# tum-vision/lsd_slam

Measured on AMD Instinct MI355X. Metric: tracked frames/sec (full track+map loop) at 640x480, frames resident in HBM (8-bit upload excluded: value_pcie_inclusive has it), higher is better.
Workload: dtype f32

## Files before the change

lsd_slam_amd/csrc/lsdhip_internal.hpp:

```cpp
#pragma once
#include <hip/hip_runtime.h>
#include <atomic>
#include <chrono>
#include <cmath>
#include <cstddef>
#include <cstdint>
#include <cstdio>
#include <cstring>
#include <mutex>
#include <string>
#include <vector>
#include "../../include/lsdhip.h"

#define LSD_LEVELS LSDHIP_PYRAMID_LEVELS
#define LSD_TRACK_MIN_LEVEL 1
#define LSD_TRACK_MAX_LEVEL 5
#define LSD_QUICK_KF_CHECK_LVL 4

void lsd_set_error(const char* fmt, ...);
#define HIPCHK(expr)                                                                       \
  do {                                                                                     \
    hipError_t e_ = (expr);                                                                \
    if (e_ != hipSuccess) {                                                                \
      lsd_set_error("%s failed: %s (%s:%d)", #expr, hipGetErrorString(e_), __FILE__, __LINE__); \
// ... 49 lines not shown
  TrackLevel lv[LSD_LEVELS];
  uint8_t* wasGood;
  float cameraPixelNoise2, var_weight, huber_half;
  float lambdaSuccessFac, lambdaFailFac;
  int useAffine;
  int lastLevel;
  int topLevel;
  lsdm::SE3fH T0;
  float aff_a0, aff_b0;
  int evalOnly;
  int trackFrameSemantics;
};
struct TrackSpec {
  int specC;
  int specGrid;
  int trials[LSD_LEVELS];
  uint8_t* wasGoodSide;
  unsigned maskStride;
  int seq;
  int copyMask;
  unsigned long long dbgCum;
  unsigned long long* dbgCounters;
  int last;
#ifdef LSD_PHASE_TRACE
  int traceWg;
#endif
#ifdef LSD_DEVTOOLS
  int* dbgLog;
#endif
};

struct TrackState {
  lsdm::SE3fH T;
  lsdm::SE3fH Tn;
  float R[9], t[3];
  float aff_a, aff_b, aff_a_lastIt, aff_b_lastIt;
  float lastErr, LM_lambda, last_residual;
  int level, iteration, incTry, phase;
  int pending;
  float A[36], b[6];
  float inc[6];
  float bytes;
  int done, diverged;
  int numEvaluations, numWarpUpdates;
  float pointUsage, goodCount, badCount, meanRes;
  int levelEvals[LSD_LEVELS];
// ... 414 lines not shown
```

lsd_slam_amd/csrc/track_device.hpp:

```cpp
#pragma once
#include "lsdhip_internal.hpp"
#include <type_traits>

template <int CTRL, int ROW_MASK, int BANK_MASK>
__device__ __forceinline__ float dpp_f(float v) {
  return __builtin_bit_cast(float, __builtin_amdgcn_update_dpp(0, __builtin_bit_cast(int, v), CTRL, ROW_MASK, BANK_MASK, true));
}
__device__ __forceinline__ int dpp_max_i(int a, int b) { return a > b ? a : b; }
template <int CTRL, int ROW_MASK, int BANK_MASK>
__device__ __forceinline__ int dpp_i(int v) {
  return __builtin_amdgcn_update_dpp(-1, v, CTRL, ROW_MASK, BANK_MASK, false);
}
template <int CTRL, int ROW_MASK, int BANK_MASK>
__device__ __forceinline__ int dpp_i0(int v) {
  return __builtin_amdgcn_update_dpp(0, v, CTRL, ROW_MASK, BANK_MASK, true);
}
__device__ __forceinline__ int wave_max_to_lane63(int v) {
  int t = dpp_max_i(v, dpp_i<0x111, 0xf, 0xf>(v));
  t = dpp_max_i(t, dpp_i<0x112, 0xf, 0xf>(v));
  t = dpp_max_i(t, dpp_i<0x113, 0xf, 0xf>(v));
  t = dpp_max_i(t, dpp_i<0x114, 0xf, 0xe>(t));
  t = dpp_max_i(t, dpp_i<0x118, 0xf, 0xc>(t));
  t = dpp_max_i(t, dpp_i<0x142, 0xa, 0xf>(t));
  t = dpp_max_i(t, dpp_i<0x143, 0xc, 0xf>(t));
// ... 400 lines not shown
  float tot[RS_NUM];
};
struct LmPar {
  float lambdaInitial, stepSizeMin, convergenceEps, minWarped, lambdaSuccessFac, lambdaFailFac;
  int maxIts, w, h, writeMask, evalOnly, useAffine, tfSemantics, lastLevel, trials;
};
__device__ __forceinline__ void stage_lm_par(const TrackJob& job, int level, LmPar& p, const int trials = 1) {
  const TrackLevel& L = job.lv[level];
  LmPar v;
  v.lambdaInitial = L.lambdaInitial; v.stepSizeMin = L.stepSizeMin; v.convergenceEps = L.convergenceEps; v.minWarped = L.minWarped;
  v.lambdaSuccessFac = job.lambdaSuccessFac; v.lambdaFailFac = job.lambdaFailFac;
  v.maxIts = L.maxIts; v.w = L.w; v.h = L.h; v.writeMask = L.writeMask; v.evalOnly = job.evalOnly; v.useAffine = job.useAffine;
  v.tfSemantics = job.trackFrameSemantics; v.lastLevel = job.lastLevel;
  v.trials = trials;
  p = v;
}

#ifdef LSD_PHASE_TRACE
#define LM_MARK(k) do { if (trp && lane == 0) trp[k] = clock64(); } while (0)
#else
#define LM_MARK(k) do { } while (0)
#endif
__device__ __forceinline__ float lm_werr(float sumWeightedErr, int M) { return sumWeightedErr * frcp((float)((M >> 2) << 2)); }
__device__ __forceinline__ float lm_lambda_fail(float LM_lambda, int incTry, float lambdaFailFac) {
  if (LM_lambda == 0) return 0.2f;
  double p = 1.0;
  for (int i = 0; i < incTry; i++) p *= (double)lambdaFailFac;
  return (float)((double)LM_lambda * p);
}
__device__ __forceinline__ float eval_bytes(const float N, const LmPar& L) {
  const float wh = (float)L.w * (float)L.h;
  const float texels = 4.0f * N < wh ? 4.0f * N : wh;
  return 20.0f * N + (L.writeMask ? 5.0f * N : 0.0f) + 12.0f * texels;
}
__device__ __forceinline__ float inc_norm2(const float* inc) {
  const float i0 = inc[0], i1 = inc[1], i2 = inc[2], i3 = inc[3], i4 = inc[4], i5 = inc[5];
  return (i0 * i0 + (i1 * i1 + i2 * i2)) + (i3 * i3 + (i4 * i4 + i5 * i5));
}
template <bool SPEC = false>
__device__ __forceinline__ bool lm_wave(const LmPar& par, TrackState& S, const float col, LmShared& sh, const int lane,
                                        TrackSummary* out, unsigned long long* trp, const int consumed = 0, const int mycand = 0, const int doneWord = 1) {
  float* const tot = sh.tot;
  S.lastCand = consumed;
  S.ncand = 1;
  const LmPar L = par;
  const int maxIts = L.maxIts;
  const int M = (int)rl(col, RS_M);
  const float refNum = rl(col, RS_NREF);
  const float goodCount = rl(col, RS_GOOD), badCount = rl(col, RS_BAD);
  float aff_a_lastIt, aff_b_lastIt;
  {
// ... 8 lines not shown
  S.meanRes = rl(col, RS_SUMSIGNED) * frcp(goodCount);
  S.aff_a_lastIt = aff_a_lastIt;
  S.aff_b_lastIt = aff_b_lastIt;
  S.numEvaluations = S.numEvaluations + 1;
  if (lane == 0) S.levelEvals[S.level] = S.levelEvals[S.level] + 1;
  S.bytes = S.bytes + eval_bytes(refNum, L);
  S.pending = 0;
  LM_MARK(12);
  if (L.evalOnly) { S.done = 1; if (out && lane == 0) write_summary(S, tot, out, doneWord); return false; }

  if (M < L.minWarped) {
    S.diverged = 1; S.done = 1;
    if (out && lane == 0) write_summary(S, tot, out, doneWord);
    return false;
  }
  const float werr = lm_werr(rl(col, RS_WERR), M);
  const bool useAffine = L.useAffine != 0;
  const bool tfSemantics = L.tfSemantics != 0;

  float LM_lambda = S.LM_lambda, lastErr = S.lastErr;
  int iteration = S.iteration, incTry = S.incTry;
  lsdm::SE3fH T = S.T;
  bool propose = false, start_iteration = false, accepted = false, rejected = false;
  if (S.phase == 0) {
    accepted = true;
    lastErr = werr;
    LM_lambda = L.lambdaInitial;
    iteration = 0;
    start_iteration = true;
  } else {
    const float error = werr;
    if (error < lastErr) {
      accepted = true;
      T = S.Tn;
      S.T = T;
      if (error > L.convergenceEps * lastErr) iteration = maxIts;
      lastErr = error;
      if (tfSemantics) S.last_residual = error;
      if (LM_lambda <= 0.2) LM_lambda = 0;
      else LM_lambda *= L.lambdaSuccessFac;
      iteration++;
      start_iteration = true;
    } else {
      if (!(inc_norm2(S.inc) > L.stepSizeMin)) {
        iteration = maxIts;
        iteration++;
        start_iteration = true;
      } else {
        LM_lambda = lm_lambda_fail(LM_lambda, incTry, L.lambdaFailFac);
        propose = true;
        rejected = true;
      }
    }
  }
  if (accepted) {
    if (useAffine) { S.aff_a = aff_a_lastIt; S.aff_b = aff_b_lastIt; }
    const float rn = frcp((float)((size_t)6 * (size_t)(M >> 2)));
    const int k = lane - RS_A0;
    if (k >= 0 && k < 21) {
      const int i = (k >= 6) + (k >= 11) + (k >= 15) + (k >= 18) + (k >= 20);
      const int j = k - (i * 6 - (i * (i - 1)) / 2) + i;
      const float v = (0.0f + col) * rn;
      S.A[i * 6 + j] = v;
      S.A[j * 6 + i] = v;
    }
    if (lane >= RS_B0 && lane < RS_B0 + 6) S.b[lane - RS_B0] = (0.0f - col) * rn;
  }
  if (start_iteration && iteration < maxIts) { S.numWarpUpdates = S.numWarpUpdates + 1; incTry = 0; propose = true; }
  S.lastErr = lastErr;
  S.LM_lambda = LM_lambda;
  S.iteration = iteration;
  LM_MARK(13);
  if (propose) {
    const int extra = SPEC ? mycand : 0;
    for (int j = 0; j < extra; j++) { incTry++; LM_lambda = lm_lambda_fail(LM_lambda, incTry, L.lambdaFailFac); }
    S.ncand = L.trials;
    float inc[6];
    const float damp = 1 + LM_lambda;
    LM_MARK(14);
    gj6_solve_wave(S.A, S.b, damp, sh.gj, lane, inc);
    LM_MARK(15);
    S.incTry = incTry + 1;
#pragma unroll
    for (int i = 0; i < 6; i++) S.inc[i] = inc[i];
    set_eval_pose(S, se3f_mul_wave(se3f_exp_wave(inc, lane), T, lane));
    S.phase = 1;
    LM_MARK(16);
    return true;
  }
  S.incTry = incTry;
  if (!tfSemantics) S.last_residual = lastErr;
  if (S.level == L.lastLevel) {
    S.done = 1;
    if (out && lane == 0) write_summary(S, tot, out, doneWord);
  } else {
    S.level = S.level - 1;
    S.phase = 0;
    set_eval_pose(S, T);
// ... 126 lines not shown
__device__ __forceinline__ int xcd_tile(int b, int nb) { return (nb & 7) == 0 ? (b & 7) * (nb >> 3) + (b >> 3) : b; }


struct TrialRecord {
  float inc[6];
  float pose[7];
  float R[9], t[3];
  float pad_[7];
};
static_assert(sizeof(TrialRecord) == 128 && sizeof(lsdm::SE3fH) == sizeof(float[7]), "a trial record is 32 floats; its pose is a TrackState::Tn");
enum { TRIAL_RECORD_WORDS = offsetof(TrialRecord, pad_) / 4 };
__device__ __forceinline__ float trial_record_word(const TrackState& S, const int i) {
  constexpr int P = offsetof(TrialRecord, pose) / 4, R = offsetof(TrialRecord, R) / 4, T = offsetof(TrialRecord, t) / 4;
  return i < P ? S.inc[i] : (i < R ? ((const float*)&S.Tn)[i - P] : (i < T ? S.R[i - R] : S.t[i - T]));
}
__device__ __forceinline__ void trial_record_adopt(TrackState& S, const TrialRecord& rec, const int lane) {
  if (lane < 6) S.inc[lane] = rec.inc[lane];
  if (lane < 7) ((float*)&S.Tn)[lane] = rec.pose[lane];
  if (lane < 9) S.R[lane] = rec.R[lane];
  if (lane < 3) S.t[lane] = rec.t[lane];
}
__device__ __forceinline__ int trials_at(const TrackSpec& spec, const int level) { return (spec.specC > 1 && spec.trials[level] > 1) ? spec.trials[level] : 1; }

#define RS_COLS 44
struct TrackScratch {
  float* sums;
  int4* topkey;
  float* topval;
  int max_rows;
  int cmax;
  TrialRecord* recs;
#ifdef LSD_PHASE_TRACE
  unsigned long long* trace;
#endif
};
```

lsd_slam_amd/csrc/tracker.hip:

```cpp
#include <atomic>
#include <chrono>
#include "track_device.hpp"
#include "reposition_plan.hpp"

#ifdef LSD_PHASE_TRACE
#define PHASE_MARK(k) do { if (trOn_ && threadIdx.x == 0) tr_[k] = clock64(); } while (0)
#define LSD_TRACE_WORDS 32
#define TRACE_PARAMS , const bool trOn_, unsigned long long* const tr_
#define TRACE_ARGS , trOn_, tr_
#define TRACE_PUT(rec, who, k, v) do { if (trOn_ && threadIdx.x == (who)) (rec)[k] = (unsigned long long)(v); } while (0)
#define TRACE_LM_REC (trOn_ ? tr_ : nullptr)
__device__ __forceinline__ unsigned long long* trace_open(unsigned long long* trace, const bool mine, unsigned long long** s_trp) {
  if (!mine) return trace;
  const unsigned long long n = trace[0];
  trace[0] = n + 1;
  unsigned long long* tr_ = trace + 1 + (n % 4096) * LSD_TRACE_WORDS;
  for (int k = 0; k < LSD_TRACE_WORDS; k++) tr_[k] = 0;
  tr_[8] = wall_clock64();
  tr_[24] = (unsigned long long)gridDim.x; tr_[25] = (unsigned long long)gridDim.y;
  *s_trp = tr_;
  return tr_;
}
#else
#define PHASE_MARK(k) do { } while (0)
// ... 31 lines not shown
  if (tid < 36) S.A[tid] = 0;
  if (tid < 6) { S.b[tid] = 0; S.inc[tid] = 0; }
}

struct StepAddr {
  const float *sums_in, *topval_in;
  float *sums_out, *topval_out;
  const int4* topkey_in; int4* topkey_out;
  const TrialRecord* recs_in;
  TrialRecord* recs_out;
  int max_rows, cmax;
};
template <bool BATCH, int MODE>
__device__ __forceinline__ StepAddr step_addr(const TrackScratch& sc, const int parity) {
  const size_t rows = (size_t)sc.max_rows, cm = (size_t)sc.cmax, job0 = BATCH ? (size_t)blockIdx.y * 2 * cm : 0;
  const size_t in = job0 + (size_t)parity * cm, out = job0 + (size_t)(MODE == TS_EVAL ? parity : 1 - parity) * cm;
  constexpr size_t TAIL = TAIL_ROWS * TAIL_STRIDE;
  return {sc.sums + in * RS_COLS * rows, sc.topval + in * rows * TAIL, sc.sums + out * RS_COLS * rows, sc.topval + out * rows * TAIL,
          sc.topkey + in * rows, sc.topkey + out * rows, sc.recs + in, sc.recs + out, sc.max_rows, sc.cmax};
}

struct StepRole { int cand, bx; bool leader, leaves; };
template <bool BATCH, int MODE>
__device__ __forceinline__ void step_role(StepRole& r, const TrackJob& job, const TrackSpec& spec, const TrackState& S) {
  const int lvlPending = S.level;
  if (MODE == TS_FUSED) {
    const int nbl = job.lv[lvlPending].nblocks;
    const int tr = trials_at(spec, lvlPending);
    r.cand = (int)blockIdx.x / nbl; r.bx = (int)blockIdx.x - r.cand * nbl;
    const bool needTrial = S.pending ? r.cand < tr : r.cand == 0;
    const bool needNext = S.pending && lvlPending > job.lastLevel && (int)blockIdx.x < job.lv[lvlPending - 1].nblocks;
    r.leaves = !r.leader && !needTrial && !needNext;
  }
  if (BATCH && MODE == TS_LM) {
    r.cand = (int)blockIdx.x; r.bx = 0;
    r.leaves = !r.leader && !(S.pending && r.cand < trials_at(spec, lvlPending));
  }
  if (BATCH && MODE == TS_EVAL) {
    const int nbl = job.lv[lvlPending].nblocks;
    r.cand = (int)blockIdx.x / nbl; r.bx = (int)blockIdx.x - r.cand * nbl;
  }
}

constexpr int STRIP_CHMAX = 8;
__device__ __forceinline__ void strip_request(const TrackLevel& L, const int tile_, const int wave, const int lane, int& cntv, unsigned (&ow)[STRIP_CHMAX]) {
  const int px = L.w * L.h;
  const int base_ = tile_ * L.tilePx;
  const int b0_ = base_ >> 8;
  const int mblk_ = (min(base_ + L.tilePx, px) - base_ + 255) >> 8;
  const gbyte* offs = (const gbyte*)L.kf_refBlk;
  const __attribute__((address_space(1))) int* cnts = (const __attribute__((address_space(1))) int*)(offs + ((size_t)((px + 255) >> 8) << 8));
  cntv = lane < mblk_ ? cnts[b0_ + lane] : 0;
#pragma unroll
  for (int c = 0; c < STRIP_CHMAX; c++) {
    const int blk = c * 4 + wave;
    ow[c] = blk < mblk_ ? *(const __attribute__((address_space(1))) unsigned*)(offs + ((size_t)(b0_ + blk) << 8) + (lane << 2)) : 0u;
  }
}

// ... 166 lines not shown
      a4.w += live ? v[c][q].w : 0.f;
    }
    if (sumLane && base + c < ncandPending) *(float4*)&s_sumT[base + c][slot][c4 * 4] = a4;
  }
}
template <int TRIALS_MAX>
__device__ __forceinline__ void column_sums(const StepAddr& A, const int nb, const int ncandPending, const int t, const SumTable s_sumT) {
  constexpr int NSLOT = SUM_NSLOT, QMAX = SUM_QMAX;
  const int slot_ = t / (RS_COLS / 4); const bool sumLane = slot_ < NSLOT;
  const int slot = sumLane ? slot_ : 0, c4 = sumLane ? t - slot_ * (RS_COLS / 4) : 0;
  const int K = (nb + NSLOT - 1) / NSLOT;
  const float4* p = (const float4*)A.sums_in + c4;
  const size_t trialStrideF4 = (size_t)RS_COLS * A.max_rows / 4;
  if (ncandPending == 1) {
    if (K <= 2) colsum<2, 1>(p, trialStrideF4, nb, ncandPending, 0, slot, c4, sumLane, s_sumT);
    else if (K <= 5) colsum<5, 1>(p, trialStrideF4, nb, ncandPending, 0, slot, c4, sumLane, s_sumT);
    else if (K <= 10) colsum<10, 1>(p, trialStrideF4, nb, ncandPending, 0, slot, c4, sumLane, s_sumT);
    else colsum<QMAX, 1>(p, trialStrideF4, nb, ncandPending, 0, slot, c4, sumLane, s_sumT);
  } else if (K <= 2) colsum<2, TRIALS_MAX>(p, trialStrideF4, nb, ncandPending, 0, slot, c4, sumLane, s_sumT);
  else if (K <= 5) colsum<5, TRIALS_MAX>(p, trialStrideF4, nb, ncandPending, 0, slot, c4, sumLane, s_sumT);
  else if (K <= 10) { for (int base = 0; base < ncandPending; base += 3) colsum<10, 3>(p, trialStrideF4, nb, ncandPending, base, slot, c4, sumLane, s_sumT); }
  else { for (int base = 0; base < ncandPending; base++) colsum<QMAX, 1>(p, trialStrideF4, nb, ncandPending, base, slot, c4, sumLane, s_sumT); }
}
template <int TRIALS_MAX>
struct FinishTables {
  enum { WORDS = TRIALS_MAX * (SUM_NSLOT * RS_COLS + TAIL_ROWS * TAIL_STRIDE + 1) };
  SumTable sum; TailTable sub; int* nsub;
  __device__ __forceinline__ explicit FinishTables(float* buf)
      : sum((SumTable)buf), sub((TailTable)(buf + TRIALS_MAX * SUM_NSLOT * RS_COLS)), nsub((int*)(buf + TRIALS_MAX * (SUM_NSLOT * RS_COLS + TAIL_ROWS * TAIL_STRIDE))) {}
};
__device__ __forceinline__ float slot_total(const SumTable s_sumT, const int c, const int col) {
  float s = s_sumT[c][0][col];
#pragma unroll
  for (int k = 1; k < SUM_NSLOT; k++) s += s_sumT[c][k][col];
  return s;
}

__device__ __forceinline__ int pick_trial(TrackState& S, const LmPar& par, const int level, const int ncandPending, const SumTable s_sumT, const TailTable s_subT,
                                          const int* s_nsubT, const TrialRecord* s_rec, const int tid) {
  if (ncandPending <= 1) return 0;
  const int c = tid < ncandPending ? tid : 0;
  const int Mc = (int)slot_total(s_sumT, c, RS_M);
  const float ws = tail_drop(slot_total(s_sumT, c, RS_WERR), Mc, s_nsubT[c], tail_word(RS_WERR), s_subT[c]);
  const float werrc = lm_werr(ws, Mc);
  const float incdot = inc_norm2(c == 0 ? S.inc : s_rec[c].inc);
  const bool stop = Mc < par.minWarped || werrc < S.lastErr || !(incdot > par.stepSizeMin);
  const unsigned long long sm = __ballot(stop && tid < ncandPending);
  const int pc = sm ? (int)__ffsll((long long)sm) - 1 : ncandPending - 1;
  if (pc > 0) {
    float lam = S.LM_lambda;
    const int it0 = S.incTry;
    for (int j = 0; j < pc; j++) lam = lm_lambda_fail(lam, it0 + j, par.lambdaFailFac);
    const float skipped = eval_bytes(slot_total(s_sumT, 0, RS_NREF), par);
    const float bytes0 = S.bytes;
    const int ne0 = S.numEvaluations, le0 = S.levelEvals[level];
    float bytes1 = bytes0;
    for (int j = 0; j < pc; j++) bytes1 = bytes1 + skipped;
    S.LM_lambda = lam;
    S.incTry = it0 + pc;
    S.numEvaluations = ne0 + pc;
    if (tid == 0) S.levelEvals[level] = le0 + pc;
    S.bytes = bytes1;
    trial_record_adopt(S, s_rec[pc], tid);
  }
  return pc;
}
__device__ __forceinline__ float finish_totals(const SumTable s_sumT, const TailTable s_subT, const int* s_nsubT, const int pc, const int tid) {
  const int M = (int)slot_total(s_sumT, pc, RS_M);
  const float s = tid < RS_END ? slot_total(s_sumT, pc, tid) : 0.f;
  return tail_drop(s, M, s_nsubT[pc], tail_word(tid), s_subT[pc]);
}
template <int BLOCK>
__device__ __forceinline__ void copy_side_mask(const TrackJob& job, const TrackState& S, const TrackSpec& spec, const int level, const int bx, const int nb, const int tid) {
  const uint8_t* side = spec.wasGoodSide + (size_t)(S.lastCand - 1) * spec.maskStride;
  EvalCtx a;
  make_ctx_dev(job, S, level, a);
  const int work = a.npts >= 0 ? a.npts : a.w * a.h;
  for (int i = bx * BLOCK + tid; i < work; i += nb * BLOCK) {
    float px, py, pz, I_ref, var;
    int maskIdx;
    if (fetch_point(a, i, px, py, pz, I_ref, var, maskIdx) && maskIdx >= 0) job.wasGood[maskIdx] = side[maskIdx];
  }
}

template <int BLOCK>
__device__ __forceinline__ void eval_strip(const EvalCtx& a, const int tilePx, const int tile, const int work, const int cntv, const unsigned (&ow)[STRIP_CHMAX],
                                           unsigned* const s_list , gbyte* const wasGood, float (&acc)[RS_END], int& key0, int& key1, int& key2,
                                           const int tid TRACE_PARAMS) {
  const int wave = tid >> 6, lane = tid & 63;
  const int base = tile * tilePx;
  const int stripEnd = min(base + tilePx, work);
  const int b0 = base >> 8;
// ... 45 lines not shown
    stageA(tid, A1);
    stageB(A1, B0);
    stageA(tid + BLOCK, A1);
    PHASE_MARK(22);
    auto stageC = [&](const StB& B) {
      if (B.live) {
        const int x_ = (int)(B.xy & 0xffffu), y_ = (int)(B.xy >> 16);
        visit_point(a, B.q, B.t, B.pz, B.I_ref, B.var, wasGood, __mul24(y_, a.w) + x_, __mul24(x_, a.h) + y_, acc, key0, key1, key2);
      }
    };
    for (int r = 0; r < rounds; r += 2) {
      stageB(A1, B1);
      stageA(tid + (r + 2) * BLOCK, A2);
      stageC(B0);
      stageB(A2, B0);
      stageA(tid + (r + 3) * BLOCK, A1);
      stageC(B1);
    }
  }
  __syncthreads();
}
__device__ __forceinline__ void eval_groups_of_four(const EvalCtx& a, int i, const int stride, const int work, gbyte* const wasGood, float (&acc)[RS_END],
                                                    int& key0, int& key1, int& key2) {
  const int sy = stride / a.w, sx = stride - sy * a.w;
  int x = i % a.w, y = i / a.w;
  struct Pt { int i, x, y; bool valid; RefPlanes r; float img, pz; PointWarp q; PointTexels t; };
  while (i < work) {
    Pt P[4];
#pragma unroll
    for (int k = 0; k < 4; k++) {
      Pt& p = P[k];
      p.i = i; p.x = x; p.y = y;
      p.valid = i < work;
      const int li = p.valid ? i : 0;
      fetch_request(a, li, p.r);
      p.img = a.kf_image[li];
      i += stride; x += sx; y += sy;
      if (x >= a.w) { x -= a.w; y++; }
    }
#pragma unroll
    for (int k = 0; k < 4; k++) {
      Pt& p = P[k];
      float px = 0.f, py = 0.f;
      p.pz = 1.f;
      p.valid = p.valid && ref_pixel_inside(a, p.x, p.y) && fetch_finish(a, p.x, p.y, p.r, px, py, p.pz);
      eval_warp(a, px, py, p.pz, p.q);
      eval_fetch(a, p.q, p.valid && p.q.in_image, p.t);
    }
// ... 15 lines not shown
      if (q.in_image) eval_fetch(a, q, true, t);
      visit_point(a, q, t, pz, I_ref, var, maskIdx >= 0 ? wasGood : nullptr, maskIdx, a.npts >= 0 ? i : (i % a.w) * a.h + (i / a.w), acc, key0, key1, key2);
    }
  }
}

constexpr int RED_NPASS = 1;
constexpr int RED_CPP = (RS_END + RED_NPASS - 1) / RED_NPASS;
template <int BLOCK, bool BATCH, int MODE>
__device__ __forceinline__ void reduce_and_store(const EvalCtx& a, const TrackLevel& L, TrackState& S, const int tile, const float (&acc)[RS_END],
                                                 const int key0, const int key1, const int key2, float* const s_red, float (*const s_sum)[64], int (*const s_wtop)[3],
                                                 int* const s_top, float* const sums_out, int4* const topkey_out, float* const topval_out, const int tid) {
  constexpr int NPASS = RED_NPASS, CPP = RED_CPP;
  constexpr int RSLICE = BLOCK / CPP;
  constexpr int RRUN = (BLOCK + RSLICE - 1) / RSLICE;
  const bool stripRows = BATCH && L.tilePx > 0;
  const bool candLane = tid >= BLOCK - 64 && tid < BLOCK - 61;
  TailCandidate c;
  float cPz = 0.f;
  PointWarp cq; PointTexels ct;
  if (stripRows) {
    block_top3(key0, key1, key2, s_wtop, s_top);
    if (candLane) c.request(a, s_top[tid - (BLOCK - 64)]);
  }
#pragma unroll
  for (int hp = 0; hp < NPASS; hp++) {
    if (hp > 0) __syncthreads();
#pragma unroll
    for (int k = 0; k < CPP; k++)
      if (hp * CPP + k < RS_END) s_red[k * (BLOCK + 1) + tid] = acc[hp * CPP + k];
    __syncthreads();
    if (MODE == TS_FUSED && hp == 0 && tid == 0) { S.pending = 1; S.numLaunches = S.numLaunches + 1; }
    if (stripRows && hp == 0 && candLane && c.key >= 0) {
      float px, py;
      ref_point_at(a, c.x, c.y, c.id, px, py, cPz);
      eval_warp(a, px, py, cPz, cq);
      eval_fetch(a, cq, cq.in_image, ct);
    }
    {
      const int slice = tid / CPP, k = tid - slice * CPP;
      if (slice < RSLICE) s_sum[slice][k] = slice_sum<BLOCK + 1, RRUN>(s_red, k, slice);
    }
    __syncthreads();
    if (stripRows && hp == 0 && candLane) {
      float* row = topval_out + (size_t)(tile * TAIL_ROWS + (tid - (BLOCK - 64))) * TAIL_STRIDE;
      if (c.key >= 0) {
        PointOut o;
        eval_finish(a, cq, ct, cPz, c.img, c.var, o);
        tail_row(o, row);
      }
      ((int*)row)[TAIL_KEY] = c.key;
    }
    if (tid < CPP && hp * CPP + tid < RS_END) {
      float s = s_sum[0][tid];
#pragma unroll
      for (int sl = 1; sl < RSLICE; sl++) s += s_sum[sl][tid];
      sums_out[(size_t)tile * RS_COLS + (hp * CPP + tid)] = s;
    }
  }
  if (!stripRows) block_top3(key0, key1, key2, s_wtop, s_top);
  if (tid == 0) topkey_out[tile] = make_int4(s_top[0], s_top[1], s_top[2], -1);
  if (L.singlePass && key0 >= 0) {
    const int r = key0 == s_top[0] ? 0 : (key0 == s_top[1] ? 1 : (key0 == s_top[2] ? 2 : -1));
    if (r >= 0) tail_row_from_sums(acc, topval_out + (size_t)(tile * TAIL_ROWS + r) * TAIL_STRIDE);
  }
}

#ifdef LSD_ORDER_CHECK
__device__ __forceinline__ void order_check_totals(const TrackSpec& spec, const float s, const int pc, const int tid) {
  unsigned hv = tid < RS_END ? __float_as_uint(s) * (2654435761u * (unsigned)(tid + 1)) : 0u;
  hv += (unsigned)pc * 97u;
  for (int off = 32; off > 0; off >>= 1) hv += __shfl_xor(hv, off);
  if (tid == 0) {
    const unsigned long long slot = 8 + 2 * ((spec.dbgCum / 400ull) % 8192ull);
    __hip_atomic_fetch_min(&spec.dbgCounters[slot], (unsigned long long)hv, __ATOMIC_RELAXED, __HIP_MEMORY_SCOPE_AGENT);
    __hip_atomic_fetch_max(&spec.dbgCounters[slot + 1], (unsigned long long)hv, __ATOMIC_RELAXED, __HIP_MEMORY_SCOPE_AGENT);
  }
}
#endif

__device__ __forceinline__ void warm_job_arguments() {
  typedef const unsigned __attribute__((address_space(4))) cuint;
  cuint* ka = (cuint*)__builtin_amdgcn_kernarg_segment_ptr();
  unsigned warm = 0;
#pragma unroll
  for (int i = 0; i < (int)(sizeof(TrackJob) / 4); i += 32) warm ^= ka[i];
  asm volatile("" ::"s"(warm));
}

template <int BLOCK, bool BATCH, int MODE>
__device__ __forceinline__ void track_step_impl(const TrackJob& jobv, const TrackJob* __restrict__ jobs, TrackState* __restrict__ st2,
                                                TrackScratch sc, TrackSummary* __restrict__ out, int parity, int first, const TrackSpec& spec) {
  const TrackJob& job = BATCH ? jobs[blockIdx.y] : jobv;
  if (!BATCH) warm_job_arguments();
  if (BATCH) { st2 += 2 * (size_t)blockIdx.y; out += blockIdx.y; }
  const StepAddr A = step_addr<BATCH, MODE>(sc, parity);
  constexpr int WAVES = BLOCK / 64, SUMW = WAVES - 1;
  constexpr int NSLICE = (SUMW * 64) / RS_END, CPP = RED_CPP, RSLICE_ = BLOCK / CPP;
  __shared__ TrackState S;
  __shared__ LmShared sh;
  __shared__ LmPar s_par;
  __shared__ float s_sum[(NSLICE > RSLICE_ ? NSLICE : RSLICE_)][64];
  __shared__ __attribute__((aligned(16))) float s_red[CPP * (BLOCK + 1) + 8];
  __shared__ int s_wtop[WAVES][3];
  __shared__ int s_top[3];
  const int tid = threadIdx.x, wave = tid >> 6, lane = tid & 63;
  StepRole role = {0, (int)blockIdx.x, blockIdx.x == 0, false};
  const bool leader = role.leader;
  TrackState* next = st2 + (1 - parity);
  constexpr int TRIALS_MAX = BATCH ? (MODE == TS_EVAL ? 1 : LSD_BATCH_SPEC_MAX) : LSD_SPEC_MAX;
  constexpr bool SPEC_LM = MODE != TS_EVAL;
  static_assert(FinishTables<TRIALS_MAX>::WORDS <= CPP * (BLOCK + 1) + 8, "the finishing phase's tables must fit the reduction buffer");
  const FinishTables<TRIALS_MAX> ft(s_red);
  __shared__ TrialRecord s_rec[TRIALS_MAX];
#ifdef LSD_PHASE_TRACE
  __shared__ unsigned long long* s_trp;
  const bool trOn_ = sc.trace != nullptr && (int)blockIdx.x == (BATCH ? spec.traceWg : 0) && (!BATCH || blockIdx.y == 0);
  unsigned long long* const tr_ = trace_open(sc.trace, trOn_ && tid == 0, &s_trp);
#endif
  PHASE_MARK(0);
  if (!BATCH && MODE == TS_FUSED && !first && !leader && st2[parity].done) return;
  if (!BATCH && MODE == TS_FUSED && leader && tid == 0 && spec.seq != 0) out->seq = spec.seq;
  if (first) {
    track_state_begin(S, job, tid);
  } else {
    copy_words<sizeof(TrackState) / 4>(&S, st2 + parity, tid, BLOCK);
    if (SPEC_LM && A.cmax > 1 && tid < (int)(sizeof(s_rec) / 4)) ((float*)s_rec)[tid] = ((const float*)A.recs_in)[tid < (int)(sizeof(TrialRecord) / 4) * A.cmax ? tid : 0];
  }
  __syncthreads();
  PHASE_MARK(1);
#ifdef LSD_DEVTOOLS
  const int lvlIn_ = S.level, numLaunchesIn_ = S.numLaunches, pendingIn_ = S.pending, ncandIn_ = S.ncand;
#endif
  if (S.done) {
    LAUNCH_LOG(1, pendingIn_, ncandIn_, -1);
    if (MODE != TS_EVAL && leader) { copy_words<sizeof(TrackState) / 4>(next, &S, tid, BLOCK); }
    return;
  }
  const int lvlPending = S.level;
  const int doneWord = (MODE == TS_FUSED && spec.seq != 0) ? (BATCH ? spec.seq : (spec.seq >> 12)) : 1;
  step_role<BATCH, MODE>(role, job, spec, S);
  if (role.leaves) return;
  int cand = role.cand, bx = role.bx;

  int cntv = 0;
  unsigned ow[STRIP_CHMAX];
  bool havePre = false;
  if (BATCH && MODE == TS_FUSED && S.pending && job.lv[lvlPending].tilePx > 0) {
    havePre = cand < trials_at(spec, lvlPending);
    if (havePre) strip_request(job.lv[lvlPending], xcd_tile(bx, job.lv[lvlPending].nblocks), wave, lane, cntv, ow);
  }

  if (MODE != TS_EVAL && S.pending) {
    const int ncandPending = S.ncand < 1 ? 1 : (S.ncand > TRIALS_MAX ? TRIALS_MAX : S.ncand);
    const int level = S.level;
    const int nb = job.lv[level].nblocks;
    if (tid == SUMW * 64 - 1) stage_lm_par(job, level, s_par, trials_at(spec, level));
    if (wave < SUMW) {
      column_sums<TRIALS_MAX>(A, nb, ncandPending, tid, ft.sum);
      TRACE_PUT(tr_, 0, 17, clock64());
    }
    gather_tails<BATCH, WAVES>(job, S, level, nb, ncandPending, A, s_rec, ft.sub, ft.nsub, wave, lane);
    TRACE_PUT(s_trp, SUMW * 64, 18, clock64());
    __syncthreads();
    PHASE_MARK(2);
    if (wave == 0) {
      const int pc = pick_trial(S, s_par, level, ncandPending, ft.sum, ft.sub, ft.nsub, s_rec, tid);
      const float s = finish_totals(ft.sum, ft.sub, ft.nsub, pc, tid);
      if (tid < RS_NUM) sh.tot[tid] = s;
#ifdef LSD_ORDER_CHECK
      if (!BATCH && spec.dbgCounters) order_check_totals(spec, s, pc, tid);
#endif
      PHASE_MARK(3);
      TRACE_PUT(tr_, 0, 19, ncandPending); TRACE_PUT(tr_, 0, 7, pc);
      lm_wave<SPEC_LM>(s_par, S, s, sh, tid, leader ? out : nullptr, TRACE_LM_REC, pc, cand, doneWord);
    }
    __syncthreads();
    PHASE_MARK(4);
    if (S.done) {
      if (!BATCH && MODE == TS_FUSED && S.lastCand > 0 && spec.copyMask != 0 && job.lv[level].writeMask && cand == 0 && bx < nb)
        copy_side_mask<BLOCK>(job, S, spec, level, bx, nb, tid);
      if (leader) copy_words<sizeof(TrackState) / 4>(next, &S, tid, BLOCK);
      LAUNCH_LOG(2, pendingIn_, ncandIn_, S.lastCand);
      return;
    }
    if (cand > 0 && bx == 0 && S.phase == 1 && cand < S.ncand && tid < TRIAL_RECORD_WORDS) ((float*)&A.recs_out[cand])[tid] = trial_record_word(S, tid);
  }

  if (MODE == TS_LM) {
    __syncthreads();
    if (tid == 0) { S.pending = 1; S.numLaunches = S.numLaunches + 1; }
    __syncthreads();
    if (leader) copy_words<sizeof(TrackState) / 4>(next, &S, tid, BLOCK);
    return;
  }

  const int level = S.level;
  const TrackLevel& L = job.lv[level];
  const int nb = L.nblocks;
  if (MODE == TS_FUSED && level != lvlPending) { cand = 0; bx = (int)blockIdx.x; }
  if (bx >= nb || cand >= S.ncand) return;
  const int tile = xcd_tile(bx, nb);
  EvalCtx a;
  make_ctx_dev(job, S, level, a);
  if (BATCH && MODE == TS_EVAL && cand > 0) ctx_set_pose(a, A.recs_in[cand]);
  gbyte* wasGood = (gbyte*)(L.writeMask ? (cand == 0 ? job.wasGood : spec.wasGoodSide + (size_t)(cand - 1) * spec.maskStride) : nullptr);
  const int work = a.npts >= 0 ? a.npts : a.w * a.h;
  float acc[RS_END];
#pragma unroll
  for (int k = 0; k < RS_END; k++) acc[k] = 0.f;
  int key0 = -1, key1 = -1, key2 = -1;
  if (BATCH && L.tilePx > 0) {
    if (!(havePre && level == lvlPending)) strip_request(L, tile, wave, lane, cntv, ow);
    eval_strip<BLOCK>(a, L.tilePx, tile, work, cntv, ow, (unsigned*)s_red , wasGood, acc, key0, key1, key2, tid TRACE_ARGS);
  } else if (!BATCH && L.evalBatch != 0) {
    eval_groups_of_four(a, tile * BLOCK + tid, nb * BLOCK, work, wasGood, acc, key0, key1, key2);
  } else {
    eval_plain(a, tile * BLOCK + tid, nb * BLOCK, work, wasGood, acc, key0, key1, key2);
  }
  PHASE_MARK(5);
  TRACE_PUT(tr_, 0, 10, level); TRACE_PUT(tr_, 0, 11, nb); TRACE_PUT(tr_, 0, 26, lvlPending);
  reduce_and_store<BLOCK, BATCH, MODE>(a, L, S, tile, acc, key0, key1, key2, s_red, s_sum, s_wtop, s_top, A.sums_out + (size_t)cand * RS_COLS * A.max_rows,
                                       A.topkey_out + (size_t)cand * A.max_rows, A.topval_out + (size_t)cand * A.max_rows * (TAIL_ROWS * TAIL_STRIDE), tid);
  if (MODE == TS_FUSED && leader) copy_words<sizeof(TrackState) / 4>(next, &S, tid, BLOCK);
  if (MODE == TS_FUSED && leader && tid == 0 && spec.last != 0) out->exhausted = spec.seq;
  LAUNCH_LOG(3, pendingIn_, ncandIn_, S.lastCand);
  PHASE_MARK(6);
  TRACE_PUT(tr_, 0, 9, wall_clock64());
}

template <int BLOCK, bool BATCH, int MODE = TS_FUSED>
__global__ __launch_bounds__(BLOCK) void k_track_step(TrackJob jobv, const TrackJob* __restrict__ jobs, TrackState* __restrict__ st2,
                                                       TrackScratch sc, TrackSummary* __restrict__ out, int parity, int first, TrackSpec spec) {
#ifdef LSD_ORDER_CHECK
  if (!BATCH && spec.dbgCounters && threadIdx.x == 0) {
    const unsigned long long fin = __hip_atomic_load(&spec.dbgCounters[0], __ATOMIC_RELAXED, __HIP_MEMORY_SCOPE_AGENT);
    if (fin < spec.dbgCum) {
      __hip_atomic_fetch_add(&spec.dbgCounters[1], 1ull, __ATOMIC_RELAXED, __HIP_MEMORY_SCOPE_AGENT);
// ... 718 lines not shown
struct DevTime {};
inline DevTime dev_now() { return {}; }
inline void dev_log_pointer(lsdhip_tracker*, TrackSpec&) {}
inline void dev_job_begins(lsdhip_tracker*) {}
inline void dev_launches_queued(lsdhip_tracker*, int, DevTime) {}
inline void dev_budget_missed(lsdhip_tracker*) {}
struct DevWaitClock { explicit DevWaitClock(lsdhip_tracker*) {} };
inline int dev_dump_first_launch(lsdhip_tracker*, const TrackJob&, int, int) { return LSDHIP_OK; }
inline int dev_keep_launch_log(lsdhip_tracker*) { return LSDHIP_OK; }
inline void dev_trace_job(lsdhip_ctx*, const lsdhip_frame*, const lsdhip_frame*, const double*) {}
inline void dev_trace_launched(lsdhip_tracker*, int, const lsdhip_frame*) {}
inline void dev_trace_result(lsdhip_tracker*, int, const lsdhip_frame*) {}
inline int dev_replay_check(lsdhip_tracker*, TrackJob&, const lsdhip_frame*, const lsdhip_frame*, const lsdm::SE3fH&, lsdm::SE3fH*, int rc) { return rc; }
#endif

static int launch_seq(const lsdhip_tracker* t) { return t->jobTag ? ((t->jobTag << 12) | (t->launchOrdinal & 0xFFF)) : 0; }
static void launch_step(lsdhip_tracker* t, const TrackJob& job, TrackSpec spec, int grid, int parity, int first, int last) {
  lsdhip_ctx* c = t->ctx;
  LSD_CTX_LOCK(c);
  TrackScratch sc = scratch_of(t);
  t->launchOrdinal++;
  spec.seq = launch_seq(t);
  spec.last = last;
  dev_log_pointer(t, spec);
#ifdef LSD_ORDER_CHECK
  spec.dbgCum = t->dbgCum;
  spec.dbgCounters = t->d_dbg;
  t->dbgCum += (unsigned long long)grid;
#endif
  hipLaunchKernelGGL((k_track_step<256, false>), dim3(grid), dim3(256), 0, c->stream, job, (const TrackJob*)nullptr, t->d_state, sc,
                     t->d_summary, parity, first, spec);
}
static int launch_steps(lsdhip_tracker* t, const TrackJob& job, const TrackSpec& spec, int grid, int steps, int* parity, int* first) {
  const DevTime tl0 = dev_now();
  for (int i = 0; i < steps; i++) {
    launch_step(t, job, spec, grid, *parity, *first, i + 1 == steps);
    lsdhip_host_mark(20);
    *first = 0;
    *parity ^= 1;
  }
  dev_launches_queued(t, steps, tl0);
  HIPCHK(hipGetLastError());
  return LSDHIP_OK;
}
struct EvalOut {
  int warped_size;
// ... 193 lines not shown
  LevelWork lv[LSD_LEVELS];
  SpecPolicy p;
  p.specC = t->specC; p.specAuto = t->specAuto; p.specCap = t->specCap; p.grid_cap = t->grid_cap; p.block = t->block;
  for (int l = 0; l < LSD_LEVELS; l++) {
    const TrackLevel& L = job.lv[l];
    lv[l] = {L.npts >= 0 ? (long long)L.npts : (long long)L.w * L.h, {L.nblocks, L.singlePass, L.tilePx}};
    p.specLevel[l] = t->specLevel[l]; p.specCaps[l] = t->specCaps[l];
  }
  const SinglePlan P = lsd_single_plan(lv, p, job.lastLevel, job.topLevel);
  for (int l = 0; l < LSD_LEVELS; l++) {
    job.lv[l].nblocks = P.tiling[l].nblocks; job.lv[l].singlePass = P.tiling[l].singlePass;
    job.lv[l].evalBatch = eval_batch_level(t, job.lv[l]);
  }
  return P;
}
static TrackSpec job_spec(const lsdhip_tracker* t, const SinglePlan& P) {
  TrackSpec spec = TrackSpec{};
  spec.specC = t->specC;
  spec.specGrid = P.specGrid;
  for (int l = 0; l < LSD_LEVELS; l++) spec.trials[l] = P.trials[l];
  spec.wasGoodSide = side_planes(t);
  spec.maskStride = (unsigned)t->maskStride;
  spec.copyMask = t->ctx->pipeline ? 0 : 1;
  return spec;
}

static int track_device(lsdhip_tracker* t, TrackJob& job, int topLevel, const lsdm::SE3fH& T0, lsdm::SE3fH* Tout) {
  lsdhip_ctx* c = t->ctx;
  job.evalOnly = 0;
  job.topLevel = topLevel;
  job.T0 = T0;
  job.aff_a0 = 1.0f; job.aff_b0 = 0.0f;
  if (int rc = claim_side_planes(t)) return rc;
  const SinglePlan plan = plan_job(t, job);
  const TrackSpec spec = job_spec(t, plan);
  TrackSummary* S = t->h_summary;
  volatile const int* done = &S->done;
  S->done = 0;
  const long long myEpoch = ++c->enqEpoch;
  const bool sample = c->prof_on && ((c->prof_tick++ & 7) == 0);
  dev_job_begins(t);
  t->jobTag = (t->jobTag % 0x7FFFF) + 1;
  t->launchOrdinal = 0;
  S->seq = 0;
  S->exhausted = 0;
  int parity = 0, first = 1;
// ... 744 lines not shown
```

Measured before the change: 5712.

## Pack per-level tiles and trials into launch args and trim tracker step latency

Per-level tile counts and trial counts are packed into 64-bit and 32-bit spec fields, so the non-batched fused step can derive its role from scalar kernel arguments instead of indexing the job struct. The state load is issued before the early-done check, per-trial slot totals are computed once into a shared table in parallel, the lambda failure power is computed incrementally, pixel coordinates use a reciprocal-based split, and the per-block top-3 merge for non-strip evaluation moves into the reduction pass. These changes target latency in the small, latency-bound LM step kernels, at the cost of more shared memory, an extra barrier, and 12-bit/4-bit packing limits on tile and trial counts.

Result: faster. 6036 (median of 6 runs) (+5.7%).

```diff
diff --git a/lsd_slam_amd/csrc/lsdhip_internal.hpp b/lsd_slam_amd/csrc/lsdhip_internal.hpp
--- a/lsd_slam_amd/csrc/lsdhip_internal.hpp
+++ b/lsd_slam_amd/csrc/lsdhip_internal.hpp
@@ -95,6 +95,8 @@
   unsigned long long dbgCum;
   unsigned long long* dbgCounters;
   int last;
+  unsigned long long levelTiles;
+  unsigned levelTrials;
 #ifdef LSD_PHASE_TRACE
   int traceWg;
 #endif
diff --git a/lsd_slam_amd/csrc/track_device.hpp b/lsd_slam_amd/csrc/track_device.hpp
--- a/lsd_slam_amd/csrc/track_device.hpp
+++ b/lsd_slam_amd/csrc/track_device.hpp
@@ -446,11 +446,14 @@
 #define LM_MARK(k) do { } while (0)
 #endif
 __device__ __forceinline__ float lm_werr(float sumWeightedErr, int M) { return sumWeightedErr * frcp((float)((M >> 2) << 2)); }
-__device__ __forceinline__ float lm_lambda_fail(float LM_lambda, int incTry, float lambdaFailFac) {
-  if (LM_lambda == 0) return 0.2f;
+__device__ __forceinline__ double lambda_fail_pow(int incTry, float lambdaFailFac) {
   double p = 1.0;
   for (int i = 0; i < incTry; i++) p *= (double)lambdaFailFac;
-  return (float)((double)LM_lambda * p);
+  return p;
+}
+__device__ __forceinline__ float lm_lambda_fail_pow(float LM_lambda, double pow_incTry) { return LM_lambda == 0 ? 0.2f : (float)((double)LM_lambda * pow_incTry); }
+__device__ __forceinline__ float lm_lambda_fail(float LM_lambda, int incTry, float lambdaFailFac) {
+  return lm_lambda_fail_pow(LM_lambda, lambda_fail_pow(incTry, lambdaFailFac));
 }
 __device__ __forceinline__ float eval_bytes(const float N, const LmPar& L) {
   const float wh = (float)L.w * (float)L.h;
@@ -505,6 +508,7 @@
   int iteration = S.iteration, incTry = S.incTry;
   lsdm::SE3fH T = S.T;
   bool propose = false, start_iteration = false, accepted = false, rejected = false;
+  double failPow = 1.0;
   if (S.phase == 0) {
     accepted = true;
     lastErr = werr;
@@ -530,7 +534,8 @@
         iteration++;
         start_iteration = true;
       } else {
-        LM_lambda = lm_lambda_fail(LM_lambda, incTry, L.lambdaFailFac);
+        failPow = lambda_fail_pow(incTry, L.lambdaFailFac);
+        LM_lambda = lm_lambda_fail_pow(LM_lambda, failPow);
         propose = true;
         rejected = true;
       }
@@ -549,14 +554,14 @@
     }
     if (lane >= RS_B0 && lane < RS_B0 + 6) S.b[lane - RS_B0] = (0.0f - col) * rn;
   }
-  if (start_iteration && iteration < maxIts) { S.numWarpUpdates = S.numWarpUpdates + 1; incTry = 0; propose = true; }
+  if (start_iteration && iteration < maxIts) { S.numWarpUpdates = S.numWarpUpdates + 1; incTry = 0; failPow = 1.0; propose = true; }
   S.lastErr = lastErr;
   S.LM_lambda = LM_lambda;
   S.iteration = iteration;
   LM_MARK(13);
   if (propose) {
     const int extra = SPEC ? mycand : 0;
-    for (int j = 0; j < extra; j++) { incTry++; LM_lambda = lm_lambda_fail(LM_lambda, incTry, L.lambdaFailFac); }
+    for (int j = 0; j < extra; j++) { incTry++; failPow *= (double)L.lambdaFailFac; LM_lambda = lm_lambda_fail_pow(LM_lambda, failPow); }
     S.ncand = L.trials;
     float inc[6];
     const float damp = 1 + LM_lambda;
@@ -729,6 +734,12 @@
 }
 __device__ __forceinline__ int trials_at(const TrackSpec& spec, const int level) { return (spec.specC > 1 && spec.trials[level] > 1) ? spec.trials[level] : 1; }
 
+struct LevelFacts {
+  unsigned long long tiles; unsigned trials; int lastLevel;
+  __device__ __forceinline__ int tiles_at(const int level) const { return (int)(tiles >> (12 * level)) & 0xFFF; }
+  __device__ __forceinline__ int trials_at(const int level) const { return (int)(trials >> (4 * level)) & 0xF; }
+};
+
 #define RS_COLS 44
 struct TrackScratch {
   float* sums;
diff --git a/lsd_slam_amd/csrc/tracker.hip b/lsd_slam_amd/csrc/tracker.hip
--- a/lsd_slam_amd/csrc/tracker.hip
+++ b/lsd_slam_amd/csrc/tracker.hip
@@ -77,19 +77,28 @@
 
 struct StepRole { int cand, bx; bool leader, leaves; };
 template <bool BATCH, int MODE>
-__device__ __forceinline__ void step_role(StepRole& r, const TrackJob& job, const TrackSpec& spec, const TrackState& S) {
-  const int lvlPending = S.level;
-  if (MODE == TS_FUSED) {
+__device__ __forceinline__ void step_role(StepRole& r, const TrackJob& job, const TrackSpec& spec, const LevelFacts& lf, const int lvlPending, const int pending) {
+  if (MODE == TS_FUSED && !BATCH) {
+    const int nbl = lf.tiles_at(lvlPending), tr = lf.trials_at(lvlPending);
+    int cand = 0;
+#pragma unroll
+    for (int k = 1; k <= LSD_SPEC_MAX; k++) cand += (int)blockIdx.x >= k * nbl ? 1 : 0;
+    r.cand = cand; r.bx = (int)blockIdx.x - cand * nbl;
+    const bool needTrial = pending ? cand < tr : cand == 0;
+    const bool needNext = pending && lvlPending > lf.lastLevel && (int)blockIdx.x < lf.tiles_at(lvlPending > 0 ? lvlPending - 1 : 0);
+    r.leaves = !r.leader && !needTrial && !needNext;
+  }
+  if (MODE == TS_FUSED && BATCH) {
     const int nbl = job.lv[lvlPending].nblocks;
     const int tr = trials_at(spec, lvlPending);
     r.cand = (int)blockIdx.x / nbl; r.bx = (int)blockIdx.x - r.cand * nbl;
-    const bool needTrial = S.pending ? r.cand < tr : r.cand == 0;
-    const bool needNext = S.pending && lvlPending > job.lastLevel && (int)blockIdx.x < job.lv[lvlPending - 1].nblocks;
+    const bool needTrial = pending ? r.cand < tr : r.cand == 0;
+    const bool needNext = pending && lvlPending > job.lastLevel && (int)blockIdx.x < job.lv[lvlPending - 1].nblocks;
     r.leaves = !r.leader && !needTrial && !needNext;
   }
   if (BATCH && MODE == TS_LM) {
     r.cand = (int)blockIdx.x; r.bx = 0;
-    r.leaves = !r.leader && !(S.pending && r.cand < trials_at(spec, lvlPending));
+    r.leaves = !r.leader && !(pending && r.cand < trials_at(spec, lvlPending));
   }
   if (BATCH && MODE == TS_EVAL) {
     const int nbl = job.lv[lvlPending].nblocks;
@@ -302,12 +311,14 @@
   else if (K <= 10) { for (int base = 0; base < ncandPending; base += 3) colsum<10, 3>(p, trialStrideF4, nb, ncandPending, base, slot, c4, sumLane, s_sumT); }
   else { for (int base = 0; base < ncandPending; base++) colsum<QMAX, 1>(p, trialStrideF4, nb, ncandPending, base, slot, c4, sumLane, s_sumT); }
 }
+typedef float (*TotalTable)[RS_COLS];
 template <int TRIALS_MAX>
 struct FinishTables {
-  enum { WORDS = TRIALS_MAX * (SUM_NSLOT * RS_COLS + TAIL_ROWS * TAIL_STRIDE + 1) };
-  SumTable sum; TailTable sub; int* nsub;
+  enum { WORDS = TRIALS_MAX * (SUM_NSLOT * RS_COLS + TAIL_ROWS * TAIL_STRIDE + 1 + RS_COLS) };
+  SumTable sum; TailTable sub; int* nsub; TotalTable tot;
   __device__ __forceinline__ explicit FinishTables(float* buf)
-      : sum((SumTable)buf), sub((TailTable)(buf + TRIALS_MAX * SUM_NSLOT * RS_COLS)), nsub((int*)(buf + TRIALS_MAX * (SUM_NSLOT * RS_COLS + TAIL_ROWS * TAIL_STRIDE))) {}
+      : sum((SumTable)buf), sub((TailTable)(buf + TRIALS_MAX * SUM_NSLOT * RS_COLS)), nsub((int*)(buf + TRIALS_MAX * (SUM_NSLOT * RS_COLS + TAIL_ROWS * TAIL_STRIDE))),
+        tot((TotalTable)(buf + TRIALS_MAX * (SUM_NSLOT * RS_COLS + TAIL_ROWS * TAIL_STRIDE + 1))) {}
 };
 __device__ __forceinline__ float slot_total(const SumTable s_sumT, const int c, const int col) {
   float s = s_sumT[c][0][col];
@@ -315,13 +326,19 @@
   for (int k = 1; k < SUM_NSLOT; k++) s += s_sumT[c][k][col];
   return s;
 }
-
-__device__ __forceinline__ int pick_trial(TrackState& S, const LmPar& par, const int level, const int ncandPending, const SumTable s_sumT, const TailTable s_subT,
+template <int TRIALS_MAX, int BLOCK>
+__device__ __forceinline__ void slot_totals(const SumTable s_sumT, const TotalTable s_totT, const int ncandPending, const int tid) {
+  static_assert(TRIALS_MAX * RS_END <= BLOCK, "a thread per (trial, column)");
+  const int c = tid / RS_END, col = tid - c * RS_END;
+  if (c < ncandPending) s_totT[c][col] = slot_total(s_sumT, c, col);
+}
+
+__device__ __forceinline__ int pick_trial(TrackState& S, const LmPar& par, const int level, const int ncandPending, const TotalTable s_totT, const TailTable s_subT,
                                           const int* s_nsubT, const TrialRecord* s_rec, const int tid) {
   if (ncandPending <= 1) return 0;
   const int c = tid < ncandPending ? tid : 0;
-  const int Mc = (int)slot_total(s_sumT, c, RS_M);
-  const float ws = tail_drop(slot_total(s_sumT, c, RS_WERR), Mc, s_nsubT[c], tail_word(RS_WERR), s_subT[c]);
+  const int Mc = (int)s_totT[c][RS_M];
+  const float ws = tail_drop(s_totT[c][RS_WERR], Mc, s_nsubT[c], tail_word(RS_WERR), s_subT[c]);
   const float werrc = lm_werr(ws, Mc);
   const float incdot = inc_norm2(c == 0 ? S.inc : s_rec[c].inc);
   const bool stop = Mc < par.minWarped || werrc < S.lastErr || !(incdot > par.stepSizeMin);
@@ -330,8 +347,9 @@
   if (pc > 0) {
     float lam = S.LM_lambda;
     const int it0 = S.incTry;
-    for (int j = 0; j < pc; j++) lam = lm_lambda_fail(lam, it0 + j, par.lambdaFailFac);
-    const float skipped = eval_bytes(slot_total(s_sumT, 0, RS_NREF), par);
+    double failPow = lambda_fail_pow(it0, par.lambdaFailFac);
+    for (int j = 0; j < pc; j++) { lam = lm_lambda_fail_pow(lam, failPow); failPow *= (double)par.lambdaFailFac; }
+    const float skipped = eval_bytes(s_totT[0][RS_NREF], par);
     const float bytes0 = S.bytes;
     const int ne0 = S.numEvaluations, le0 = S.levelEvals[level];
     float bytes1 = bytes0;
@@ -345,9 +363,9 @@
   }
   return pc;
 }
-__device__ __forceinline__ float finish_totals(const SumTable s_sumT, const TailTable s_subT, const int* s_nsubT, const int pc, const int tid) {
-  const int M = (int)slot_total(s_sumT, pc, RS_M);
-  const float s = tid < RS_END ? slot_total(s_sumT, pc, tid) : 0.f;
+__device__ __forceinline__ float finish_totals(const TotalTable s_totT, const TailTable s_subT, const int* s_nsubT, const int pc, const int tid) {
+  const int M = (int)s_totT[pc][RS_M];
+  const float s = tid < RS_END ? s_totT[pc][tid] : 0.f;
   return tail_drop(s, M, s_nsubT[pc], tail_word(tid), s_subT[pc]);
 }
 template <int BLOCK>
@@ -439,8 +457,10 @@
 }
 __device__ __forceinline__ void eval_groups_of_four(const EvalCtx& a, int i, const int stride, const int work, gbyte* const wasGood, float (&acc)[RS_END],
                                                     int& key0, int& key1, int& key2) {
-  const int sy = stride / a.w, sx = stride - sy * a.w;
-  int x = i % a.w, y = i / a.w;
+  const float inv_w = frcp((float)a.w);
+  const unsigned sxy = pixel_xy16(stride, a.w, inv_w), ixy = pixel_xy16(i, a.w, inv_w);
+  const int sy = (int)(sxy >> 16), sx = (int)(sxy & 0xFFFFu);
+  int x = (int)(ixy & 0xFFFFu), y = (int)(ixy >> 16);
   struct Pt { int i, x, y; bool valid; RefPlanes r; float img, pz; PointWarp q; PointTexels t; };
   while (i < work) {
     Pt P[4];
@@ -502,6 +522,8 @@
   if (stripRows) {
     block_top3(key0, key1, key2, s_wtop, s_top);
     if (candLane) c.request(a, s_top[tid - (BLOCK - 64)]);
+  } else {
+    wave_top3(key0, key1, key2, s_wtop);
   }
 #pragma unroll
   for (int hp = 0; hp < NPASS; hp++) {
@@ -521,6 +543,13 @@
       const int slice = tid / CPP, k = tid - slice * CPP;
       if (slice < RSLICE) s_sum[slice][k] = slice_sum<BLOCK + 1, RRUN>(s_red, k, slice);
     }
+    if (!stripRows && hp == 0 && tid >= BLOCK - 64) {
+      int top[3];
+      merge_top3(s_wtop, BLOCK / 64, top);
+#pragma unroll
+      for (int r = 0; r < 3; r++)
+        if (tid == BLOCK - 64) s_top[r] = top[r];
+    }
     __syncthreads();
     if (stripRows && hp == 0 && candLane) {
       float* row = topval_out + (size_t)(tile * TAIL_ROWS + (tid - (BLOCK - 64))) * TAIL_STRIDE;
@@ -538,7 +567,6 @@
       sums_out[(size_t)tile * RS_COLS + (hp * CPP + tid)] = s;
     }
   }
-  if (!stripRows) block_top3(key0, key1, key2, s_wtop, s_top);
   if (tid == 0) topkey_out[tile] = make_int4(s_top[0], s_top[1], s_top[2], -1);
   if (L.singlePass && key0 >= 0) {
     const int r = key0 == s_top[0] ? 0 : (key0 == s_top[1] ? 1 : (key0 == s_top[2] ? 2 : -1));
@@ -575,6 +603,11 @@
   if (!BATCH) warm_job_arguments();
   if (BATCH) { st2 += 2 * (size_t)blockIdx.y; out += blockIdx.y; }
   const StepAddr A = step_addr<BATCH, MODE>(sc, parity);
+  LevelFacts lf = {0ull, 0u, 0};
+  if (!BATCH) {
+    lf = {spec.levelTiles, spec.levelTrials, job.lastLevel};
+    asm volatile("" ::"s"(lf.tiles), "s"(lf.trials), "s"(lf.lastLevel));
+  }
   constexpr int WAVES = BLOCK / 64, SUMW = WAVES - 1;
   constexpr int NSLICE = (SUMW * 64) / RS_END, CPP = RED_CPP, RSLICE_ = BLOCK / CPP;
   __shared__ TrackState S;
@@ -595,47 +628,55 @@
   __shared__ TrialRecord s_rec[TRIALS_MAX];
 #ifdef LSD_PHASE_TRACE
   __shared__ unsigned long long* s_trp;
-  const bool trOn_ = sc.trace != nullptr && (int)blockIdx.x == (BATCH ? spec.traceWg : 0) && (!BATCH || blockIdx.y == 0);
+  const bool trOn_ = sc.trace != nullptr && (int)blockIdx.x == spec.traceWg && (!BATCH || blockIdx.y == 0);
   unsigned long long* const tr_ = trace_open(sc.trace, trOn_ && tid == 0, &s_trp);
 #endif
   PHASE_MARK(0);
-  if (!BATCH && MODE == TS_FUSED && !first && !leader && st2[parity].done) return;
   if (!BATCH && MODE == TS_FUSED && leader && tid == 0 && spec.seq != 0) out->seq = spec.seq;
   if (first) {
     track_state_begin(S, job, tid);
   } else {
-    copy_words<sizeof(TrackState) / 4>(&S, st2 + parity, tid, BLOCK);
-    if (SPEC_LM && A.cmax > 1 && tid < (int)(sizeof(s_rec) / 4)) ((float*)s_rec)[tid] = ((const float*)A.recs_in)[tid < (int)(sizeof(TrialRecord) / 4) * A.cmax ? tid : 0];
+    constexpr int NSTATE = (int)(sizeof(TrackState) / 4), NREC = (int)(sizeof(s_rec) / 4);
+    static_assert(NSTATE <= BLOCK && NREC <= BLOCK, "one word of the state and one of the records per thread");
+    const bool haveRecs = SPEC_LM && A.cmax > 1;
+    const unsigned stateWord = ((const unsigned*)(st2 + parity))[tid < NSTATE ? tid : 0];
+    float recWord = 0.f;
+    if (haveRecs) recWord = ((const float*)A.recs_in)[tid < (int)(sizeof(TrialRecord) / 4) * A.cmax && tid < NREC ? tid : 0];
+    if (!BATCH && MODE == TS_FUSED && !leader && st2[parity].done) return;
+    if (tid < NSTATE) ((unsigned*)&S)[tid] = stateWord;
+    if (haveRecs && tid < NREC) ((float*)s_rec)[tid] = recWord;
   }
   __syncthreads();
   PHASE_MARK(1);
 #ifdef LSD_DEVTOOLS
   const int lvlIn_ = S.level, numLaunchesIn_ = S.numLaunches, pendingIn_ = S.pending, ncandIn_ = S.ncand;
 #endif
-  if (S.done) {
+  const int doneIn = S.done, lvlPending = S.level, pending = S.pending, ncandIn = S.ncand;
+  if (doneIn) {
     LAUNCH_LOG(1, pendingIn_, ncandIn_, -1);
     if (MODE != TS_EVAL && leader) { copy_words<sizeof(TrackState) / 4>(next, &S, tid, BLOCK); }
     return;
   }
-  const int lvlPending = S.level;
   const int doneWord = (MODE == TS_FUSED && spec.seq != 0) ? (BATCH ? spec.seq : (spec.seq >> 12)) : 1;
-  step_role<BATCH, MODE>(role, job, spec, S);
+  step_role<BATCH, MODE>(role, job, spec, lf, lvlPending, pending);
   if (role.leaves) return;
   int cand = role.cand, bx = role.bx;
+  PHASE_MARK(20);
 
   int cntv = 0;
   unsigned ow[STRIP_CHMAX];
   bool havePre = false;
-  if (BATCH && MODE == TS_FUSED && S.pending && job.lv[lvlPending].tilePx > 0) {
+  if (BATCH && MODE == TS_FUSED && pending && job.lv[lvlPending].tilePx > 0) {
     havePre = cand < trials_at(spec, lvlPending);
     if (havePre) strip_request(job.lv[lvlPending], xcd_tile(bx, job.lv[lvlPending].nblocks), wave, lane, cntv, ow);
   }
 
-  if (MODE != TS_EVAL && S.pending) {
-    const int ncandPending = S.ncand < 1 ? 1 : (S.ncand > TRIALS_MAX ? TRIALS_MAX : S.ncand);
-    const int level = S.level;
-    const int nb = job.lv[level].nblocks;
-    if (tid == SUMW * 64 - 1) stage_lm_par(job, level, s_par, trials_at(spec, level));
+  int levelNow = lvlPending, ncandNow = ncandIn;
+  if (MODE != TS_EVAL && pending) {
+    const int ncandPending = ncandIn < 1 ? 1 : (ncandIn > TRIALS_MAX ? TRIALS_MAX : ncandIn);
+    const int level = lvlPending;
+    const int nb = BATCH ? job.lv[level].nblocks : lf.tiles_at(level);
+    if (tid == SUMW * 64 - 1) stage_lm_par(job, level, s_par, BATCH ? trials_at(spec, level) : lf.trials_at(level));
     if (wave < SUMW) {
       column_sums<TRIALS_MAX>(A, nb, ncandPending, tid, ft.sum);
       TRACE_PUT(tr_, 0, 17, clock64());
@@ -644,9 +685,11 @@
     TRACE_PUT(s_trp, SUMW * 64, 18, clock64());
     __syncthreads();
     PHASE_MARK(2);
+    slot_totals<TRIALS_MAX, BLOCK>(ft.sum, ft.tot, ncandPending, tid);
+    __syncthreads();
     if (wave == 0) {
-      const int pc = pick_trial(S, s_par, level, ncandPending, ft.sum, ft.sub, ft.nsub, s_rec, tid);
-      const float s = finish_totals(ft.sum, ft.sub, ft.nsub, pc, tid);
+      const int pc = pick_trial(S, s_par, level, ncandPending, ft.tot, ft.sub, ft.nsub, s_rec, tid);
+      const float s = finish_totals(ft.tot, ft.sub, ft.nsub, pc, tid);
       if (tid < RS_NUM) sh.tot[tid] = s;
 #ifdef LSD_ORDER_CHECK
       if (!BATCH && spec.dbgCounters) order_check_totals(spec, s, pc, tid);
@@ -657,14 +700,16 @@
     }
     __syncthreads();
     PHASE_MARK(4);
-    if (S.done) {
-      if (!BATCH && MODE == TS_FUSED && S.lastCand > 0 && spec.copyMask != 0 && job.lv[level].writeMask && cand == 0 && bx < nb)
+    const int doneNow = S.done, lastCandNow = S.lastCand, phaseNow = S.phase;
+    levelNow = S.level; ncandNow = S.ncand;
+    if (doneNow) {
+      if (!BATCH && MODE == TS_FUSED && lastCandNow > 0 && spec.copyMask != 0 && job.lv[level].writeMask && cand == 0 && bx < nb)
         copy_side_mask<BLOCK>(job, S, spec, level, bx, nb, tid);
       if (leader) copy_words<sizeof(TrackState) / 4>(next, &S, tid, BLOCK);
       LAUNCH_LOG(2, pendingIn_, ncandIn_, S.lastCand);
       return;
     }
-    if (cand > 0 && bx == 0 && S.phase == 1 && cand < S.ncand && tid < TRIAL_RECORD_WORDS) ((float*)&A.recs_out[cand])[tid] = trial_record_word(S, tid);
+    if (cand > 0 && bx == 0 && phaseNow == 1 && cand < ncandNow && tid < TRIAL_RECORD_WORDS) ((float*)&A.recs_out[cand])[tid] = trial_record_word(S, tid);
   }
 
   if (MODE == TS_LM) {
@@ -675,25 +720,28 @@
     return;
   }
 
-  const int level = S.level;
+  const int level = levelNow;
   const TrackLevel& L = job.lv[level];
-  const int nb = L.nblocks;
+  const int nb = BATCH ? L.nblocks : lf.tiles_at(level);
   if (MODE == TS_FUSED && level != lvlPending) { cand = 0; bx = (int)blockIdx.x; }
-  if (bx >= nb || cand >= S.ncand) return;
-  const int tile = xcd_tile(bx, nb);
   EvalCtx a;
   make_ctx_dev(job, S, level, a);
+  const int writeMask = L.writeMask, evalBatch = L.evalBatch, tilePx = L.tilePx;
+  if (bx >= nb || cand >= ncandNow) return;
+  const int tile = xcd_tile(bx, nb);
   if (BATCH && MODE == TS_EVAL && cand > 0) ctx_set_pose(a, A.recs_in[cand]);
-  gbyte* wasGood = (gbyte*)(L.writeMask ? (cand == 0 ? job.wasGood : spec.wasGoodSide + (size_t)(cand - 1) * spec.maskStride) : nullptr);
+  gbyte* wasGood = (gbyte*)(writeMask ? (cand == 0 ? job.wasGood : spec.wasGoodSide + (size_t)(cand - 1) * spec.maskStride) : nullptr);
   const int work = a.npts >= 0 ? a.npts : a.w * a.h;
   float acc[RS_END];
 #pragma unroll
   for (int k = 0; k < RS_END; k++) acc[k] = 0.f;
   int key0 = -1, key1 = -1, key2 = -1;
-  if (BATCH && L.tilePx > 0) {
+  PHASE_MARK(21);
+  TRACE_PUT(tr_, 0, 22, cand);
+  if (BATCH && tilePx > 0) {
     if (!(havePre && level == lvlPending)) strip_request(L, tile, wave, lane, cntv, ow);
-    eval_strip<BLOCK>(a, L.tilePx, tile, work, cntv, ow, (unsigned*)s_red , wasGood, acc, key0, key1, key2, tid TRACE_ARGS);
-  } else if (!BATCH && L.evalBatch != 0) {
+    eval_strip<BLOCK>(a, tilePx, tile, work, cntv, ow, (unsigned*)s_red , wasGood, acc, key0, key1, key2, tid TRACE_ARGS);
+  } else if (!BATCH && evalBatch != 0) {
     eval_groups_of_four(a, tile * BLOCK + tid, nb * BLOCK, work, wasGood, acc, key0, key1, key2);
   } else {
     eval_plain(a, tile * BLOCK + tid, nb * BLOCK, work, wasGood, acc, key0, key1, key2);
@@ -1458,6 +1506,11 @@
   t->launchOrdinal++;
   spec.seq = launch_seq(t);
   spec.last = last;
+  spec.levelTiles = 0; spec.levelTrials = 0;
+  for (int l = 0; l < LSD_LEVELS; l++) {
+    spec.levelTiles |= (unsigned long long)(job.lv[l].nblocks & 0xFFF) << (12 * l);
+    spec.levelTrials |= (unsigned)((spec.specC > 1 && spec.trials[l] > 1) ? spec.trials[l] : 1) << (4 * l);
+  }
   dev_log_pointer(t, spec);
 #ifdef LSD_ORDER_CHECK
   spec.dbgCum = t->dbgCum;
@@ -1697,6 +1750,9 @@
   spec.wasGoodSide = side_planes(t);
   spec.maskStride = (unsigned)t->maskStride;
   spec.copyMask = t->ctx->pipeline ? 0 : 1;
+#ifdef LSD_PHASE_TRACE
+  spec.traceWg = batch_env().traceWg;
+#endif
   return spec;
 }
 
```
